# IXarea/LittleGAN

Measured on AMD Instinct MI355X. Metric: 128x128 CelebA-shaped images/sec (G+D+Adj step), higher is better.
Workload: dtype bf16; 1 GPU; C3: 128x128x3 synthetic CelebA, batch 256/GPU, bf16 MFMA conv/transposed-conv + Adjuster branch; global_batch=256, per_gpu_batch=256, image=128, cond_dim=40, parallelism=dp1, launch=eager launches

## Files before the change

littlegan_amd/_lib.py:

```python
from __future__ import annotations

import ctypes as C
import os

_HERE = os.path.dirname(os.path.abspath(__file__))
LIB_PATH = os.path.join(_HERE, "liblittlegan_hip.so")

DT_F32, DT_BF16 = 0, 1

P, I, L, F, Z = C.c_void_p, C.c_int, C.c_longlong, C.c_float, C.c_size_t

SIGNATURES = {
    "lg_abi_version": (I, []),
    "lg_last_error": (C.c_char_p, []),
    "lg_conv_pack_bytes": (Z, [I, I, I]),
    "lg_conv_pack": (I, [P, P, I, I, I, P]),
    "lg_conv2d_s2_fwd": (I, [P, P, P, P, I, I, I, I, I, I, P]),
    "lg_conv_stats_workspace_bytes": (Z, [I, I, I, I, I]),
    "lg_conv_fwd_stats_fused": (I, [I, I, I, I, I, I, I]),
    "lg_conv2d_s2_fwd_stats": (I, [P, P, P, P, P, P, I, I, I, I, I, I, P, Z, P, P]),
    "lg_conv2d_s2_dgrad_m16": (I, [P, P, P, P, P, I, I, I, I, I, I, P]),
    "lg_conv2d_s2_wgrad_m16": (I, [P, P, P, P, P, P, Z, I, I, I, I, I, I, I, P]),
    "lg_conv2d_s2_dgrad": (I, [P, P, P, I, I, I, I, I, I, P]),
    "lg_conv2d_s2_wgrad": (I, [P, P, P, P, Z, I, I, I, I, I, I, I, P]),
# ... 95 lines not shown
    "lg_gp_norm_bwd": (I, [P, P, P, P, P, P, P, P, P, P, P, Z, I, L, F, P]),
    "lg_gp_norm_dd": (I, [P, P, P, P, P, P, P, P, P, P, Z, I, L, F, P]),
    "lg_gp_heads_seed": (I, [P, P, P, I, I, I, P]),
    "lg_gp_heads_2nd": (I, [P, P, P, P, P, P, P, P, I, I, I, P]),
    "lg_diffaug_draw": (I, [P, I, I, I, I, I, P, P]),
    "lg_diffaug_workspace_bytes": (Z, [I, I]),
    "lg_diffaug_fwd": (I, [P, P, P, I, I, P, Z, P]),
    "lg_diffaug_bwd": (I, [P, P, P, I, I, P, Z, P]),
    "lg_rescale_u8": (I, [P, P, I, L, P, P]),
    "lg_soft_labels": (I, [P, P, P, I, I, I, P, P]),
    "lg_augment_drawn_u8_workspace_bytes": (Z, [I]),
    "lg_augment_drawn_u8": (I, [P, P, P, P, I, I, I, F, F, F, F, F, L, L, L, P, Z, P]),
    "lgx_diffaug_draw_gated": (I, [P, I, I, I, I, I, P, P, P]),
    "lgx_ada_init": (I, [P, F, P]),
    "lgx_ada_accumulate": (I, [P, P, I, I, P]),
    "lgx_ada_adjust": (I, [P, I, F, F, P]),
    "lgr_r1_workspace_bytes": (Z, [I, L]),
    "lgr_r1_heads_seed": (I, [P, P, I, I, P]),
    "lgr_r1_seed": (I, [P, P, P, P, P, F, P, Z, I, L, P]),
    "lgr_r1_colsum_workspace_bytes": (Z, [I, I]),
    "lgr_r1_heads_colsum": (I, [P, P, P, Z, I, I, P]),
    "lgo_heads_fwd": (I, [P, P, P, P, P, P, P, P, Z, I, I, I, P]),
    "lgo_gan_heads_loss_fwd_bwd": (I, [P, P, P, I, I, F, F, P, P, I, I, I, P]),
}


GEOM_SIGNATURES = {
    "lgeo_draw": (I, [P, I, I, I, I, I, P, P, P]),
    "lgeo_fwd": (I, [P, P, P, I, I, P]),
    "lgeo_bwd": (I, [P, P, P, I, I, P]),
}


class LittleGanHipError(RuntimeError):
    pass


_lib = None


def load():
    global _lib
    if _lib is not None:
        return _lib
    if not os.path.exists(LIB_PATH):
        raise LittleGanHipError(
            f"{LIB_PATH} not found: build it with `python -m littlegan_amd.csrc.build` "
            "(the LittleGAN hot path has no CPU fallback)")
    from .csrc import build as _build
    variant = os.environ.get("LG_LIB_VARIANT") or None
    path = _build.variant_paths(variant)[1]
    if variant is None:
        fl = _build.built_flags()
        if fl is not None and fl != " ".join(_build.FLAGS):
            raise LittleGanHipError(f"{LIB_PATH} was built with non-default flags ({fl!r}); rebuild with `python -m littlegan_amd.csrc.build`")
    elif not os.path.exists(path):
        raise LittleGanHipError(f"{path} not found: build it with LG_EXTRA_FLAGS=... python -m littlegan_amd.csrc.build --variant {variant}")
    import torch
    lib = C.CDLL(path)
    for name, (res, args) in list(SIGNATURES.items()) + list(GEOM_SIGNATURES.items()):
        fn = getattr(lib, name)
        fn.restype = res
        fn.argtypes = args
    if lib.lg_abi_version() != 1:
        raise LittleGanHipError("liblittlegan_hip.so ABI version mismatch")
    _lib = lib
    return lib


def check(rc: int, what: str):
    if rc != 0:
        msg = load().lg_last_error().decode("utf-8", "replace")
        raise LittleGanHipError(f"{what} failed (rc={rc}): {msg}")
```

littlegan_amd/csrc/build.py:

```python
import glob
import os
import subprocess
import sys
from concurrent.futures import ThreadPoolExecutor

HERE = os.path.dirname(os.path.abspath(__file__))
PKG = os.path.dirname(HERE)
SOURCES = ["capi.hip", "conv_igemm.hip", "conv_halo.hip", "conv_down3.hip", "conv_up3.hip", "n3_kernels.hip", "n3_pgemm.hip", "wgrad_igemm.hip", "pack.hip", "norm.hip", "dense.hip", "heads.hip", "loss_optim.hip", "augment.hip", "fid.hip", "fid_sqrt.hip", "wgrad_at.hip", "wgrad_at32.hip", "n3_rows.hip", "skinny_mfma.hip", "conv_up4.hip", "runtime.hip", "gp.hip", "input_u8.hip", "diffaug.hip", "pairs.hip", "ada.hip", "r1.hip", "objective.hip", "geom.hip"]
LIB = os.path.join(PKG, "liblittlegan_hip.so")
FLAGS = ["--offload-arch=gfx950", "-O3", "-fPIC", "-std=c++17", "-ffp-contract=off", "-Wall", "-Wno-unused-function",
         "-Wmissing-prototypes", "-Werror=missing-prototypes", "-Xclang", "-target-feature", "-Xclang", "-packed-fp32-ops"]


def _stale(out, deps):
    if not os.path.exists(out):
        return True
    t = os.path.getmtime(out)
    return any(os.path.getmtime(d) > t for d in deps)


def variant_paths(variant):
    if not variant:
        return os.path.join(HERE, "build"), LIB
    return os.path.join(HERE, "build_" + variant), os.path.join(PKG, f"liblittlegan_hip_{variant}.so")


def build(force=False, verbose=True, variant=None):
    hipcc = os.environ.get("HIPCC", "/opt/rocm/bin/hipcc")
    objdir, LIB = variant_paths(variant)
    if not variant and os.environ.get("LG_EXTRA_FLAGS"):
        raise SystemExit("LG_EXTRA_FLAGS needs --variant NAME: ablation builds never replace the product library")
    os.makedirs(objdir, exist_ok=True)
    inc = os.path.join(os.path.dirname(PKG), "include")
    headers = sorted(glob.glob(os.path.join(HERE, "*.h"))) + sorted(glob.glob(os.path.join(inc, "littlegan_hip*.h"))) + \
        [os.path.join(inc, "littlegan_geom.h")]

    flags = FLAGS + os.environ.get("LG_EXTRA_FLAGS", "").split()
    flag_line = " ".join(flags)
    only = [s_ for s_ in os.environ.get("LG_VARIANT_SOURCES", "").split(",") if s_] if variant else []
    base_objdir = os.path.join(HERE, "build")

    def cc(src):
        s = os.path.join(HERE, src)
        if only and src not in only:
            o = os.path.join(base_objdir, src.replace(".hip", ".o"))
            if not os.path.exists(o):
                raise SystemExit(f"{o} missing: build the product library first")
            return o
        o = os.path.join(objdir, src.replace(".hip", ".o"))
        fl = o + ".flags"
        same_flags = os.path.exists(fl) and open(fl).read() == flag_line
        if force or not same_flags or _stale(o, [s] + headers):
            cmd = [hipcc] + flags + ["-c", s, "-o", o]
            if verbose:
                print(" ".join(cmd), flush=True)
            if os.path.exists(fl):
                os.remove(fl)
            subprocess.run(cmd, check=True)
            with open(fl, "w") as f:
                f.write(flag_line)
        return o

    with ThreadPoolExecutor(max_workers=6) as ex:
        objs = list(ex.map(cc, SOURCES))
    lib_fl = os.path.join(objdir, "lib.flags")
    if force or _stale(LIB, objs) or not (os.path.exists(lib_fl) and open(lib_fl).read() == flag_line):
        cmd = [hipcc, "--offload-arch=gfx950", "-shared", "-fPIC", "-o", LIB] + objs
        if verbose:
# ... 16 lines not shown
```

littlegan_amd/csrc/norm.hip:

```cpp
#include <stdio.h>
#include "lg_internal.h"
#include "philox.h"

namespace {

constexpr int CHUNK = 4096;
constexpr int EW_UNR = 4;

__global__ __launch_bounds__(256) void stats_partial_kernel(const float* __restrict__ x, double* __restrict__ partial,
                                                            long long L, int nchunk, int pre_leaky, float alpha,
                                                            __bf16* __restrict__ x16out) {
  const int n = blockIdx.y, ch = blockIdx.x;
  const long long base = (long long)n * L + (long long)ch * CHUNK;
  const long long lim = L - (long long)ch * CHUNK;
  __shared__ double sred[32];
  f32x4 v[4];
  double s = 0.0;
  int cnt = 0;
#pragma unroll
  for (int q = 0; q < 4; ++q) {
    const int e = (q * 256 + threadIdx.x) * 4;
    v[q] = f32x4{0.f, 0.f, 0.f, 0.f};
    if (e < lim) {
      v[q] = *reinterpret_cast<const f32x4*>(x + base + e);
// ... 231 lines not shown
  const double* p = partial + (long long)n * nchunk * 2;
  double s1 = 0.0, s2 = 0.0;
  for (int i = lane; i < nchunk; i += 64) { s1 += p[i * 2]; s2 += p[i * 2 + 1]; }
  s1 = lg_wave_sum_d(s1); s2 = lg_wave_sum_d(s2);
  if (lane == 0) {
    const double sigma = (double)stats[(long long)n * LG_NSTAT + 1], s = sigma + (double)LG_IN_EPS;
    const double m1 = s1 / (double)L, m2 = s2 / (double)L / (s * sigma);
    const float m1h = (float)m1, m2h = (float)m2;
    bstats[n * 4] = m1h; bstats[n * 4 + 1] = m2h;
    bstats[n * 4 + 2] = (float)(m1 - (double)m1h); bstats[n * 4 + 3] = (float)(m2 - (double)m2h);
    gsum[n * 2] = s2 / s;
    gsum[n * 2 + 1] = s1;
  }
}

__global__ __launch_bounds__(64) void bwd_coef_kernel(const double* __restrict__ partial, const float* __restrict__ stats,
                                                      float* __restrict__ coef, long long L, int nchunk) {
  const int n = blockIdx.x, lane = threadIdx.x;
  const double* p = partial + (long long)n * nchunk * 2;
  double s1 = 0.0, s2 = 0.0;
  for (int i = lane; i < nchunk; i += 64) { s1 += p[i * 2]; s2 += p[i * 2 + 1]; }
  s1 = lg_wave_sum_d(s1); s2 = lg_wave_sum_d(s2);
  if (lane == 0) {
    const float* sp = stats + (long long)n * LG_NSTAT;
    const double sigma = (double)sp[1], s = sigma + (double)LG_IN_EPS;
    const double m1 = s1 / (double)L, m2 = s2 / (double)L / (s * sigma);
    const float m1h = (float)m1, m2h = (float)m2;
    float* o = coef + (long long)n * 8;
    o[0] = sp[0]; o[1] = sp[4]; o[2] = sp[2]; o[3] = sp[3];
    o[4] = m1h; o[5] = m2h; o[6] = (float)(m1 - (double)m1h); o[7] = (float)(m2 - (double)m2h);
  }
}

__global__ __launch_bounds__(256) void bwd_affine_grad_kernel(const double* __restrict__ gsum, float* __restrict__ dgamma,
                                                              float* __restrict__ dbeta, int B, int accumulate) {
  __shared__ double sg[256], sb[256];
  double g = 0.0, b = 0.0;
  for (int i = threadIdx.x; i < B; i += 256) { g += gsum[i * 2]; b += gsum[i * 2 + 1]; }
  sg[threadIdx.x] = g; sb[threadIdx.x] = b;
  __syncthreads();
  for (int o = 128; o > 0; o >>= 1) {
    if (threadIdx.x < o) { sg[threadIdx.x] += sg[threadIdx.x + o]; sb[threadIdx.x] += sb[threadIdx.x + o]; }
    __syncthreads();
  }
  if (threadIdx.x == 0) {
    dgamma[0] = (accumulate ? dgamma[0] : 0.f) + (float)sg[0];
    dbeta[0] = (accumulate ? dbeta[0] : 0.f) + (float)sb[0];
  }
}

template <bool DB, bool DROP>
__device__ __forceinline__ void bwd_apply_body(const float* __restrict__ x, const void* __restrict__ g, int g16,
                                               const float* __restrict__ stats, const float* __restrict__ bstats,
                                               float* __restrict__ dx, __bf16* __restrict__ dx16, long long L4,
                                               long long total4, int pre_leaky, int post_leaky, float alpha,
                                               float* __restrict__ colpart, int C4, const DropK& dk, const Geo ge) {
  const DropCtx dc = drop_begin<DROP>(dk);
  constexpr int UNR = DB ? 1 : EW_UNR;
  const unsigned stride = ge.gdx * ge.bdx * UNR, tot = (unsigned)total4, l4 = (unsigned)L4;
  f32x4 csum = {0.f, 0.f, 0.f, 0.f};
  const unsigned rb = blockIdx.x;
  const int ntrip = (int)(((unsigned long long)tot + stride - 1) / stride);
  for (int tr = 0; tr < ntrip; ++tr) {
   const unsigned long long i0l = (unsigned long long)tr * stride + rb * ge.bdx * UNR + threadIdx.x;
   if (i0l >= tot) continue;
   const unsigned i0 = (unsigned)i0l;
   f32x4 xs[UNR], gs[UNR];
#pragma unroll
   for (int u = 0; u < UNR; ++u) {
     const unsigned i = i0 + u * 256;
     if (i < tot) {
       xs[u] = lg_ld<NT_LOAD>(reinterpret_cast<const f32x4*>(x + (long long)i * 4));
       gs[u] = load_g4<NT_LOAD>(g, (long long)i * 4, g16);
     }
   }
#pragma unroll
   for (int u = 0; u < UNR; ++u) {
    const unsigned i = i0 + u * 256;
    if (i >= tot) break;
    const int n = (int)(i / l4);
    const float* sp = stats + (long long)n * LG_NSTAT;
// ... 365 lines not shown
    }
  }
}

template <bool DB, bool G16>
__global__ __launch_bounds__(256) void bwd_apply16_kernel(const __bf16* __restrict__ x, const void* __restrict__ g,
                                                          const float* __restrict__ stats, const float* __restrict__ bstats,
                                                          float* __restrict__ dx, __bf16* __restrict__ dx16, long long L8,
                                                          long long total8, int pre_leaky, int post_leaky, float alpha,
                                                          float* __restrict__ colpart, int C8) {
  bwd_apply16_body<DB, G16, false>(x, g, stats, bstats, dx, dx16, L8, total8, pre_leaky, post_leaky, alpha, colpart, C8, DropK{}, Geo{blockDim.x, gridDim.x, gridDim.y});
}
template <bool DB, bool G16>
__global__ __launch_bounds__(256) void bwd_apply16_drop_kernel(const __bf16* __restrict__ x, const void* __restrict__ g,
                                                               const float* __restrict__ stats, const float* __restrict__ bstats,
                                                               float* __restrict__ dx, __bf16* __restrict__ dx16, long long L8,
                                                               long long total8, float alpha, float* __restrict__ colpart, int C8,
                                                               DropK dk) {
  bwd_apply16_body<DB, G16, true>(x, g, stats, bstats, dx, dx16, L8, total8, 0, 1, alpha, colpart, C8, dk, Geo{blockDim.x, gridDim.x, gridDim.y});
}

__global__ __launch_bounds__(256) void dropout_mask_kernel(unsigned char* __restrict__ keep, long long total8, DropK dk) {
  const DropCtx dc = drop_begin<true>(dk);
  for (long long i = (long long)blockIdx.x * 256 + threadIdx.x; i < total8; i += (long long)gridDim.x * 256) {
    float dm[8];
    drop_mult8(dc, (unsigned long long)i, dm);
    unsigned lo = 0, hi = 0;
#pragma unroll
    for (int k = 0; k < 4; ++k) { lo |= (dm[k] != 0.f ? 1u : 0u) << (8 * k); hi |= (dm[4 + k] != 0.f ? 1u : 0u) << (8 * k); }
    *reinterpret_cast<unsigned long long*>(keep + i * 8) = (unsigned long long)lo | ((unsigned long long)hi << 32);
  }
}

__global__ __launch_bounds__(1024) void colsum_final_kernel(const float* __restrict__ partial, float* __restrict__ db, int nb,
                                                            int C, int accumulate) {
  __shared__ float sr[64][17];
  const int cl = threadIdx.x & 15, gq = threadIdx.x >> 4;
  const int c = blockIdx.x * 16 + cl;
  float s = 0.f;
  if (c < C) {
    int k = gq;
    for (; k + 192 < nb; k += 256) {
      const float a = partial[(long long)k * C + c], b = partial[(long long)(k + 64) * C + c];
      const float e = partial[(long long)(k + 128) * C + c], f = partial[(long long)(k + 192) * C + c];
      s += (a + b) + (e + f);
    }
    for (; k < nb; k += 64) s += partial[(long long)k * C + c];
  }
  sr[gq][cl] = s;
  __syncthreads();
  if (gq == 0 && c < C) {
    float t = 0.f;
#pragma unroll
    for (int q = 0; q < 64; q += 4) t += (sr[q][cl] + sr[q + 1][cl]) + (sr[q + 2][cl] + sr[q + 3][cl]);
    db[c] = (accumulate ? db[c] : 0.f) + t;
  }
}

constexpr long long EW_MAX_BLOCKS = 8192;
#define LG_RESIDENT_BLOCKS(kern)                                                                                       \
  ([]() -> long long {                                                                                                 \
    static long long r = 0;                                                                                            \
    if (!r) {                                                                                                          \
      int per_cu = 0;                                                                                                  \
      if (hipOccupancyMaxActiveBlocksPerMultiprocessor(&per_cu, kern, 256, 0) != hipSuccess || per_cu < 1) per_cu = 8; \
      r = (long long)per_cu * lg_device_cus();                                                                         \
    }                                                                                                                  \
    return r;                                                                                                          \
  }())
inline long long fit_rounds(long long nb, long long resident, long long hard, int unit) {
  if (nb > hard) nb = hard;
  if (nb > resident) nb = nb / resident * resident;
  nb = nb / unit * unit;
  return nb < unit ? unit : nb;
}
inline int nchunks(long long L) { return (int)((L + CHUNK - 1) / CHUNK); }
inline int ew_blocks(long long total4) {
  long long b = (total4 + 256 * EW_UNR - 1) / (256 * EW_UNR);
  return (int)(b < EW_MAX_BLOCKS ? (b > 0 ? b : 1) : EW_MAX_BLOCKS);
}
inline size_t part_bytes(int B, long long L) { return ((size_t)B * nchunks(L) * 3 * sizeof(double) + 255) / 256 * 256; }
inline size_t bst_bytes(int B) { return ((size_t)B * 4 * sizeof(float) + 255) / 256 * 256; }

struct LaunchNote { const char* name; unsigned gx, gy; };
constexpr int NL_MAX = 8;
thread_local LaunchNote g_nl[NL_MAX];
thread_local int g_nl_n = 0;
inline void nl_reset() { g_nl_n = 0; }
inline void nl_note(const char* name, const dim3& g) {
// ... 398 lines not shown

extern "C" int lg_dropout_key(long long* key, unsigned long long seed, unsigned long long key_offset, void* stream) {
  nl_reset();
  LG_CHECK_ARG(key && ((uintptr_t)key & 7) == 0, "lg_dropout_key: null or misaligned pointer");
  NORM_LAUNCH(dropout_key_kernel, dim3(1), dim3(64), 0, (hipStream_t)stream, reinterpret_cast<unsigned long long*>(key), seed, key_offset);
  LG_CHECK_LAUNCH("lg_dropout_key");
  return LG_OK;
}

extern "C" int lg_dropout_mask(const long long* key, int call, int level, int r0, int B, long long L, float rate, unsigned char* keep,
                               void* stream) {
  nl_reset();
  LG_CHECK_ARG(keep, "lg_dropout_mask: null pointer");
  LG_CHECK_ARG(((uintptr_t)keep & 7) == 0, "lg_dropout_mask: keep must be 8-byte aligned (8 decisions per store)");
  LG_CHECK_ARG(B > 0 && L > 0 && (long long)B * L / 8 < (1LL << 31), "lg_dropout_mask: bad shape B=%d L=%lld", B, L);
  DropK dk;
  if (int rc = drop_args("lg_dropout_mask", key, call, level, r0, B, L, rate, &dk)) return rc;
  const long long total8 = (long long)B * L / 8;
  long long nb = (total8 + 255) / 256;
  if (nb > EW_MAX_BLOCKS) nb = EW_MAX_BLOCKS;
  NORM_LAUNCH(dropout_mask_kernel, dim3((int)nb), dim3(256), 0, (hipStream_t)stream, keep, total8, dk);
  LG_CHECK_LAUNCH("lg_dropout_mask");
  return LG_OK;
}

extern "C" int lg_instnorm_bwd_coef(const float* stats, const void* partials, int nparts, float* coef, int B, long long L,
                                    void* stream) {
  nl_reset();
  LG_CHECK_ARG(stats && partials && coef && nparts > 0 && B > 0 && B <= 65535 && L > 0, "lg_instnorm_bwd_coef: bad arguments");
  NORM_LAUNCH(bwd_coef_kernel, dim3(B), dim3(64), 0, (hipStream_t)stream, (const double*)partials, stats, coef, L, nparts);
  LG_CHECK_LAUNCH("lg_instnorm_bwd_coef");
  return LG_OK;
}
```

littlegan_amd/model.py:

```python
from __future__ import annotations

import math
import zlib
from typing import Dict, List, Optional

import torch

from . import ops
from ._lib import DT_BF16, DT_F32


def _dtype_of(args) -> int:
    name = getattr(args, "mfma_dtype", "f32")
    if name not in ("f32", "bf16"):
        raise ValueError(f"mfma_dtype must be 'f32' or 'bf16', got {name!r}")
    return DT_BF16 if name == "bf16" else DT_F32


def _device_of(args):
    return torch.device(getattr(args, "device", "cuda"))


def _glorot(shape, gen, device):
    if len(shape) == 2:
# ... 133 lines not shown
        r0 = 0
        if drops is not None and rows is not None:
            r0, _, step = rows.indices(ctx["enc"][0][1].shape[0])
            if step != 1:
                raise ValueError("Encoder.backward: contiguous row ranges only")
        masked = drops is not None and drops[0].active
        g_h = g_last
        levels = set(range(1, 5)) if (need_wgrad and wgrad_levels is None) else (set(wgrad_levels or ()) if need_wgrad else set())
        lowest = 1 if need_input_grad else (min(levels) if levels else 5)
        any_wgrad = need_wgrad
        nfp = None
        for i in range(4, lowest - 1, -1):
            need_wgrad = any_wgrad and i in levels
            cb, cs = self.chans[i - 1]
            x, z, st, x16 = ctx["enc"][i - 1]
            if need_wgrad and x is None and x16 is None:
                raise ValueError("Encoder.backward: this context was recorded with top_only=True (no normalised inputs kept): "
                                 "it cannot give weight gradients")
            if rows is not None:
                z, st = z[rows], st[rows]
                x = x[rows] if x is not None else None
                x16 = x16[rows] if x16 is not None else None
            dgm = self._g[f"norm{i}.gamma"] if need_wgrad else None
            dbt = self._g[f"norm{i}.beta"] if need_wgrad else None
            want_dx = i > lowest or (i == 1 and need_input_grad)
            m16 = self.dtype == DT_BF16
            if cb != 3:
                dz16 = torch.empty(z.shape, dtype=torch.bfloat16, device=z.device) if m16 else None
                drop32 = (m16 and (not need_wgrad or x16 is not None) and
                          (not want_dx or ops.conv_halo_supported(1, self.dtype, z.shape[0], z.shape[1], z.shape[2], cs, cb)))
            else:
                drop32 = m16 and ops.n3_m16_supported(z.shape[1], z.shape[2], cb, cs, self.dtype)
                dz16 = torch.empty(z.shape, dtype=torch.bfloat16, device=z.device) if drop32 else None
            dz = ops.instnorm_bwd(z, st, g_h, dgm, dbt, 0, 1, a, out16=dz16, want_f32=not drop32,
                                  db=self._g[f"conv{i}.bias"] if need_wgrad else None,
                                  partials=nfp, drop=drops[i - 1].at(r0=r0) if drops is not None else None)
            nfp = None
            if need_wgrad:
                ops.conv2d_s2_wgrad(x, dz, self._g[f"conv{i}.kernel"], False, self.dtype, x16=x16, dy16=dz16)
            if not want_dx:
                g_h = None
            elif m16 and i > 1 and drop32 and i - 1 >= lowest and not masked:
                zl, stl = ctx["enc"][i - 2][1], ctx["enc"][i - 2][2]
                if rows is not None:
                    zl, stl = zl[rows], stl[rows]
                g_h, nfp = ops.conv2d_s2_dgrad(None, packs[i - 1], cb, self.dtype, dy16=dz16, out_bf16=True, fuse=(zl, stl, a))
            else:
                g_h = ops.conv2d_s2_dgrad(dz, packs[i - 1], cb, self.dtype, dy16=dz16, out_bf16=(self.dtype == DT_BF16 and i > 1))
        return g_h if need_input_grad else None

    def backward_recorded(self, ctx, g_last):
        a = self.args.leaky_alpha
        packs = self.packs()
        rec = {}
        g_h = g_last
        for i in range(4, 0, -1):
            cb, _ = self.chans[i - 1]
            _, z, st, _ = ctx["enc"][i - 1]
            dz = ops.gp_norm_bwd(z, st, self._w[f"norm{i}.gamma"], g_h, a)
            rec[i] = (g_h, dz)
            g_h = ops.conv2d_s2_dgrad(dz, packs[i - 1], cb, self.dtype)
        return g_h, rec

    def gp_sweep(self, ctx, rec, u0, levels, lowest):
        a = self.args.leaky_alpha
        packs = self.packs()
        u_h, uz2 = u0, {}
        for i in range(1, 5):
            _, cs = self.chans[i - 1]
# ... 81 lines not shown
                h = ops.instnorm_apply(z, st, skip, 0, 1, a, out16=h16, want_f32=not drop32)
            st = ops.stats_tensor(st)
            saved.append((x, z, st, x16))
            x, x16 = h, h16
        if ctx is not None:
            ctx["dec"] = saved
        return x, x16

    def backward(self, ctx, g_h, need_wgrad: bool, wgrad_levels=None, need_input_grad: bool = True, partials=None):
        a = self.args.leaky_alpha
        packs = self.packs()
        levels = set(range(1, 5)) if (need_wgrad and wgrad_levels is None) else (set(wgrad_levels or ()) if need_wgrad else set())
        lowest = 1 if need_input_grad else (min(levels) if levels else 5)
        any_wgrad = need_wgrad
        nfp = partials
        for i in range(4, lowest - 1, -1):
            need_wgrad = any_wgrad and i in levels
            cb, cs = self.chans[i - 1]
            x, z, st, x16 = ctx["dec"][i - 1]
            dgm = self._g[f"norm{i}.gamma"] if need_wgrad else None
            dbt = self._g[f"norm{i}.beta"] if need_wgrad else None
            want_dx = i > lowest or (i == 1 and need_input_grad)
            if (not need_wgrad and want_dx and i > 1 and i - 1 >= lowest and nfp is not None and self.dtype == DT_BF16
                    and z.dtype == torch.bfloat16 and g_h.dtype == torch.bfloat16
                    and ops.convT_s2_dgrad_bn_supported(z.shape[0], z.shape[1] // 2, z.shape[2] // 2, cb, cs, self.dtype)):
                coef = ops.instnorm_bwd_coef(z, st, nfp)
                zl, stl = ctx["dec"][i - 2][1], ctx["dec"][i - 2][2]
                g_h, nfp = ops.convT_s2_dgrad_bn(z, g_h, coef, a, packs[i - 1], cs, fuse=(zl, stl, a))
                continue
            dz16 = torch.empty(z.shape, dtype=torch.bfloat16, device=z.device) if self.dtype == DT_BF16 else None
            drop32 = (dz16 is not None and (not need_wgrad or x16 is not None) and
                      ops.conv_halo_supported(0, self.dtype, z.shape[0], z.shape[1] // 2, z.shape[2] // 2, cb, cs))
            dz = ops.instnorm_bwd(z, st, g_h, dgm, dbt, 0, 1, a, out16=dz16, want_f32=not drop32,
                                  db=self._g[f"conv{i}.bias"] if need_wgrad else None, partials=nfp)
            nfp = None
            if need_wgrad:
                ops.convT_s2_wgrad(x, dz, self._g[f"conv{i}.kernel"], False, self.dtype, x16=x16, dy16=dz16)
            if not want_dx:
                g_h = None
            elif dz16 is not None and drop32 and i > 1 and i - 1 >= lowest:
                zl, stl = ctx["dec"][i - 2][1], ctx["dec"][i - 2][2]
                g_h, nfp = ops.convT_s2_dgrad(None, packs[i - 1], cs, self.dtype, dy16=dz16, out_bf16=True, fuse=(zl, stl, a))
            else:
                g_h = ops.convT_s2_dgrad(dz, packs[i - 1], cs, self.dtype, dy16=dz16, out_bf16=self.dtype == DT_BF16)
        return g_h if need_input_grad else None


class _FinalConv(_Module):

    def __init__(self, args):
        super().__init__(args)
        self.cb, self.cs = args.image_channel, args.conv_filter[4]
        self._add("kernel", (5, 5, self.cb, self.cs), "kernel")
        self._add("bias", (self.cb,), "zeros")
        self._pack = None
        self._pack_version = -1
        self.version = 0

    def pack(self):
        if self._pack_version != self.version:
            self._pack = ops.conv_pack(self._w["kernel"], self.cb, self.cs, self.dtype, out=self._pack)
            self._pack_version = self.version
        return self._pack

    def __call__(self, x, out=None, x16=None):
        return ops.convT_s1_tanh_fwd(x, self.pack(), self._w["bias"], self.cb, self.dtype, out=out, x16=x16)

# ... 328 lines not shown
```

littlegan_amd/ops.py:

```python
from __future__ import annotations

import torch

from . import _lib
from ._lib import DT_BF16, DT_F32, check

_WS = {}
_WS_RETIRED = []
_WS_PINNED = False
NSTAT = 8


class Profile:
    enabled = False
    records = []
    after_conv = None

    @classmethod
    def start(cls):
        cls.records = []
        cls.enabled = True

    @classmethod
    def stop(cls):
# ... 530 lines not shown
    if drop is not None:
        lib = _lib.load()
        if pend is not None:
            m = pend.m
            part = m.ws.data_ptr() + pend.lo * m.nparts * 3 * 8
            check(lib.lg_instnorm_leaky_apply_z16_p_drop(_p(x), part, m.nparts, _p(m.gamma), _p(m.beta), _p(stats), _p(out), _p(out16), B, Ln,
                                                         float(alpha), *drop._args(), _stream()), "lg_instnorm_leaky_apply_z16_p_drop")
            m.covered += B
        elif x_is16:
            check(lib.lg_instnorm_leaky_apply_z16_drop(_p(x), _p(stats), _p(out), _p(out16), B, Ln, float(alpha), *drop._args(), _stream()),
                  "lg_instnorm_leaky_apply_z16_drop")
        else:
            check(lib.lg_instnorm_leaky_apply_drop(_p(x), _p(stats), _p(out), _p(out16), B, Ln, float(alpha), *drop._args(), _stream()),
                  "lg_instnorm_leaky_apply_drop")
        return out
    if pend is not None:
        m = pend.m
        part = m.ws.data_ptr() + pend.lo * m.nparts * 3 * 8
        check(_lib.load().lg_instnorm_leaky_apply_z16_p(_p(x), part, m.nparts, _p(m.gamma), _p(m.beta), _p(stats), _p(skip), int(skip16),
                                                        _p(out), _p(out16), B, Ln, int(post_leaky), float(alpha), _stream()),
              "lg_instnorm_leaky_apply_z16_p")
        m.covered += B
    elif x_is16:
        check(_lib.load().lg_instnorm_leaky_apply_z16(_p(x), _p(stats), _p(skip), int(skip16), _p(out), _p(out16), B, Ln,
                                                      int(pre_leaky), int(post_leaky), float(alpha), _stream()),
              "lg_instnorm_leaky_apply_z16")
    else:
        check(_lib.load().lg_instnorm_leaky_apply(_p(x), _p(stats), _p(skip), _p(out), _p(out16), B, Ln, int(pre_leaky),
                                                  int(post_leaky), float(alpha), _stream()), "lg_instnorm_leaky_apply")
    return out


def instnorm_bwd(x, stats, g, dgamma, dbeta, pre_leaky, post_leaky, alpha, accumulate=False, out=None, out16=None,
                 want_f32=True, db=None, partials=None, drop=None):
    B = x.shape[0]
    Ln = x.numel() // B
    x_is16 = x.dtype == torch.bfloat16
    if x_is16:
        _chk16(x, x, "x")
        if Ln % 8:
            raise ValueError("instnorm_bwd: a bf16 input needs a multiple of 8 elements per sample")
    else:
        _chk(x, name="x")
    if drop is not None:
        _chk_drop(drop, "instnorm_bwd", None, pre_leaky, post_leaky, Ln)
        if partials is not None and drop.active:
            raise ValueError("instnorm_bwd: producer-fused partial sums are those of the unmasked gradient; with an active dropout "
                             "mask the first pass must run (partials=None)")
    g16 = g.dtype == torch.bfloat16
    if g16:
        _chk16(g, x, "g")
    else:
        _chk(g, name="g")
        if g.numel() != x.numel():
            raise ValueError("instnorm_bwd: g has a different size")
    _chk(stats, (B, NSTAT), "stats")
    if want_f32:
        if out is None:
            out = torch.empty(x.shape, dtype=torch.float32, device=x.device)
        _chk(out, x.shape, "out")
    else:
        if out16 is None:
            raise ValueError("instnorm_bwd: want_f32=False needs out16")
        out = None
    if out16 is not None:
        _chk16(out16, x, "out16")
    lib = _lib.load()
# ... 4 lines not shown
    ws = workspace(int(lib.lg_instnorm_bwd_db_workspace_bytes(B, Ln, C)), x.device, "small")
    if partials is not None:
        if not x_is16:
            raise ValueError("instnorm_bwd: fused partial sums belong to the bf16 activation path")
        if pre_leaky or not post_leaky or float(alpha) != partials.alpha or tuple(x.shape) != partials.shape:
            raise ValueError(f"instnorm_bwd: partial sums were produced for the post-LeakyReLU(alpha={partials.alpha}) form on "
                             f"shape {partials.shape}; asked for pre={pre_leaky} post={post_leaky} alpha={alpha} shape {tuple(x.shape)}")
        if drop is not None:
            check(lib.lg_instnorm_leaky_bwd_z16_drop(_p(x), _p(stats), _p(g), int(g16), _p(out), _p(out16), _p(dgamma), _p(dbeta), _p(db), C,
                                                     _p(partials.buf), int(partials.nparts), _p(ws), ws.numel(), B, Ln, float(alpha),
                                                     int(accumulate), *drop._args(), _stream()), "lg_instnorm_leaky_bwd_z16_drop")
            return out
        check(lib.lg_instnorm_leaky_bwd_z16_p(_p(x), _p(stats), _p(g), int(g16), _p(out), _p(out16), _p(dgamma), _p(dbeta), _p(db), C,
                                              _p(partials.buf), int(partials.nparts), _p(ws), ws.numel(), B, Ln, int(pre_leaky),
                                              int(post_leaky), float(alpha), int(accumulate), _stream()),
              "lg_instnorm_leaky_bwd_z16_p")
        return out
    if drop is not None:
        if x_is16:
            check(lib.lg_instnorm_leaky_bwd_z16_drop(_p(x), _p(stats), _p(g), int(g16), _p(out), _p(out16), _p(dgamma), _p(dbeta), _p(db), C,
                                                     None, 0, _p(ws), ws.numel(), B, Ln, float(alpha), int(accumulate), *drop._args(),
                                                     _stream()), "lg_instnorm_leaky_bwd_z16_drop")
        else:
            check(lib.lg_instnorm_leaky_bwd_drop(_p(x), _p(stats), _p(g), int(g16), _p(out), _p(out16), _p(dgamma), _p(dbeta), _p(db), C,
                                                 _p(ws), ws.numel(), B, Ln, float(alpha), int(accumulate), *drop._args(), _stream()),
                  "lg_instnorm_leaky_bwd_drop")
        return out
    fn = lib.lg_instnorm_leaky_bwd_z16 if x_is16 else lib.lg_instnorm_leaky_bwd_db
    check(fn(_p(x), _p(stats), _p(g), int(g16), _p(out), _p(out16), _p(dgamma), _p(dbeta), _p(db), C, _p(ws), ws.numel(), B, Ln,
             int(pre_leaky), int(post_leaky), float(alpha), int(accumulate), _stream()), "lg_instnorm_leaky_bwd")
    return out


def dense_fwd(x, w, bias, out=None):
    B, K = x.shape
    N = w.shape[1]
    _chk(x, name="x")
    _chk(w, (K, N), "w")
    if out is None:
        out = torch.empty(B, N, dtype=torch.float32, device=x.device)
    _chk(out, (B, N), "out")
    check(_lib.load().lg_dense_fwd(_p(x), _p(w), _p(bias), _p(out), B, K, N, _stream()), "lg_dense_fwd")
    return out


def dense_wgrad(x, dy, dw, db, accumulate=False):
    B, K = x.shape
    N = dy.shape[1]
    _chk(x, name="x")
    _chk(dy, (B, N), "dy")
    _chk(dw, (K, N), "dw")
    check(_lib.load().lg_dense_wgrad(_p(x), _p(dy), _p(dw), _p(db), B, K, N, int(accumulate), _stream()),
          "lg_dense_wgrad")


def concat_cols(a, c, out=None):
    B, ka = a.shape
    kc = c.shape[1]
    _chk(a, name="a")
    _chk(c, (B, kc), "c")
    if out is None:
        out = torch.empty(B, ka + kc, dtype=torch.float32, device=a.device)
    _chk(out, (B, ka + kc), "out")
    check(_lib.load().lg_concat_cols(_p(a), ka, _p(c), kc, _p(out), B, _stream()), "lg_concat_cols")
    return out

# ... 782 lines not shown
```

Baseline: 24800 images/sec.

## Fold instance-norm backward reductions into apply kernel and merge bias/affine tail

Adds a new instance-norm backward path for bf16 inputs. The apply kernel reduces the per-sample partial sums itself, writes the affine-gradient partials and the column bias partials, and reverses its traversal order so the most recently touched data is read first. A single tail kernel then finishes both the bias column sums and the dgamma/dbeta reduction. The aim is fewer launches and fewer separate reduction passes in the discriminator and generator backward. Each apply block now repeats the partial-sum reduction, and the path is used only when dropout is inactive.

Result: no change. 24990 images/sec (median of 6 runs) (+0.8%).

```diff
diff --git a/include/littlegan_normbwd.h b/include/littlegan_normbwd.h
--- /dev/null
+++ b/include/littlegan_normbwd.h
@@ -0,0 +1,20 @@
+#ifndef LITTLEGAN_NORMBWD_H
+#define LITTLEGAN_NORMBWD_H
+#include "littlegan_hip.h"
+
+#ifdef __cplusplus
+extern "C" {
+#endif
+
+int lgnb_bwd_z16_supported(int B, long long L, int C);
+int lgnb_plan_gx(int B, long long L, int C, long long resident);
+long long lgnb_resident_blocks(int db, int g_is_bf16);
+size_t lgnb_workspace_bytes(int B, long long L, int C);
+int lgnb_bwd_z16(const void* z16, const float* stats, const void* g, int g_is_bf16, float* dx, void* dx16, float* dgamma, float* dbeta,
+                 float* db, int C, const void* partials, int nparts_in, void* workspace, size_t ws_bytes, int B, long long L,
+                 int pre_leaky, int post_leaky, float alpha, int accumulate, void* stream);
+
+#ifdef __cplusplus
+}
+#endif
+#endif
diff --git a/littlegan_amd/_lib.py b/littlegan_amd/_lib.py
--- a/littlegan_amd/_lib.py
+++ b/littlegan_amd/_lib.py
@@ -151,6 +151,15 @@
 }
 
 
+NORMBWD_SIGNATURES = {
+    "lgnb_bwd_z16_supported": (I, [I, L, I]),
+    "lgnb_plan_gx": (I, [I, L, I, L]),
+    "lgnb_resident_blocks": (L, [I, I]),
+    "lgnb_workspace_bytes": (Z, [I, L, I]),
+    "lgnb_bwd_z16": (I, [P, P, P, I, P, P, P, P, P, I, P, I, P, Z, I, L, I, I, F, I, P]),
+}
+
+
 class LittleGanHipError(RuntimeError):
     pass
 
@@ -177,7 +186,7 @@
         raise LittleGanHipError(f"{path} not found: build it with LG_EXTRA_FLAGS=... python -m littlegan_amd.csrc.build --variant {variant}")
     import torch
     lib = C.CDLL(path)
-    for name, (res, args) in list(SIGNATURES.items()) + list(GEOM_SIGNATURES.items()):
+    for name, (res, args) in list(SIGNATURES.items()) + list(GEOM_SIGNATURES.items()) + list(NORMBWD_SIGNATURES.items()):
         fn = getattr(lib, name)
         fn.restype = res
         fn.argtypes = args
diff --git a/littlegan_amd/csrc/build.py b/littlegan_amd/csrc/build.py
--- a/littlegan_amd/csrc/build.py
+++ b/littlegan_amd/csrc/build.py
@@ -33,7 +33,7 @@
     os.makedirs(objdir, exist_ok=True)
     inc = os.path.join(os.path.dirname(PKG), "include")
     headers = sorted(glob.glob(os.path.join(HERE, "*.h"))) + sorted(glob.glob(os.path.join(inc, "littlegan_hip*.h"))) + \
-        [os.path.join(inc, "littlegan_geom.h")]
+        [os.path.join(inc, "littlegan_geom.h"), os.path.join(inc, "littlegan_normbwd.h")]
 
     flags = FLAGS + os.environ.get("LG_EXTRA_FLAGS", "").split()
     flag_line = " ".join(flags)
diff --git a/littlegan_amd/csrc/norm.hip b/littlegan_amd/csrc/norm.hip
--- a/littlegan_amd/csrc/norm.hip
+++ b/littlegan_amd/csrc/norm.hip
@@ -287,12 +287,14 @@
   }
 }
 
-__global__ __launch_bounds__(256) void bwd_affine_grad_kernel(const double* __restrict__ gsum, float* __restrict__ dgamma,
-                                                              float* __restrict__ dbeta, int B, int accumulate) {
+__device__ __forceinline__ void bwd_affine_grad_body(const double* __restrict__ gsum, float* __restrict__ dgamma,
+                                                     float* __restrict__ dbeta, int B, int accumulate) {
   __shared__ double sg[256], sb[256];
-  double g = 0.0, b = 0.0;
-  for (int i = threadIdx.x; i < B; i += 256) { g += gsum[i * 2]; b += gsum[i * 2 + 1]; }
-  sg[threadIdx.x] = g; sb[threadIdx.x] = b;
+  if (threadIdx.x < 256) {
+    double g = 0.0, b = 0.0;
+    for (int i = threadIdx.x; i < B; i += 256) { g += gsum[i * 2]; b += gsum[i * 2 + 1]; }
+    sg[threadIdx.x] = g; sb[threadIdx.x] = b;
+  }
   __syncthreads();
   for (int o = 128; o > 0; o >>= 1) {
     if (threadIdx.x < o) { sg[threadIdx.x] += sg[threadIdx.x + o]; sb[threadIdx.x] += sb[threadIdx.x + o]; }
@@ -302,6 +304,10 @@
     dgamma[0] = (accumulate ? dgamma[0] : 0.f) + (float)sg[0];
     dbeta[0] = (accumulate ? dbeta[0] : 0.f) + (float)sb[0];
   }
+}
+__global__ __launch_bounds__(256) void bwd_affine_grad_kernel(const double* __restrict__ gsum, float* __restrict__ dgamma,
+                                                              float* __restrict__ dbeta, int B, int accumulate) {
+  bwd_affine_grad_body(gsum, dgamma, dbeta, B, accumulate);
 }
 
 template <bool DB, bool DROP>
@@ -733,8 +739,8 @@
   }
 }
 
-__global__ __launch_bounds__(1024) void colsum_final_kernel(const float* __restrict__ partial, float* __restrict__ db, int nb,
-                                                            int C, int accumulate) {
+__device__ __forceinline__ void colsum_final_body(const float* __restrict__ partial, float* __restrict__ db, int nb, int C,
+                                                  int accumulate) {
   __shared__ float sr[64][17];
   const int cl = threadIdx.x & 15, gq = threadIdx.x >> 4;
   const int c = blockIdx.x * 16 + cl;
@@ -756,6 +762,10 @@
     for (int q = 0; q < 64; q += 4) t += (sr[q][cl] + sr[q + 1][cl]) + (sr[q + 2][cl] + sr[q + 3][cl]);
     db[c] = (accumulate ? db[c] : 0.f) + t;
   }
+}
+__global__ __launch_bounds__(1024) void colsum_final_kernel(const float* __restrict__ partial, float* __restrict__ db, int nb,
+                                                            int C, int accumulate) {
+  colsum_final_body(partial, db, nb, C, accumulate);
 }
 
 constexpr long long EW_MAX_BLOCKS = 8192;
@@ -1220,3 +1230,5 @@
   LG_CHECK_LAUNCH("lg_instnorm_bwd_coef");
   return LG_OK;
 }
+
+#include "norm_bwd_p.h"
diff --git a/littlegan_amd/csrc/norm_bwd_p.h b/littlegan_amd/csrc/norm_bwd_p.h
--- /dev/null
+++ b/littlegan_amd/csrc/norm_bwd_p.h
@@ -0,0 +1,219 @@
+#pragma once
+#include "../../include/littlegan_normbwd.h"
+
+namespace {
+
+constexpr int NBP_TRIPS = 2;
+
+template <bool DB, bool G16>
+__global__ __launch_bounds__(256) void bwd_apply16p_kernel(const __bf16* __restrict__ x, const void* __restrict__ g,
+                                                           const float* __restrict__ stats, const double* __restrict__ partial,
+                                                           int nchunk, double* __restrict__ gsum, float* __restrict__ dx,
+                                                           __bf16* __restrict__ dx16, unsigned L8, long long L, int pre_leaky,
+                                                           int post_leaky, float alpha, float* __restrict__ colpart, int C8) {
+  const Geo ge{blockDim.x, gridDim.x, gridDim.y};
+  constexpr int UNR = DB ? DB_UNR : EW8_UNR;
+  __shared__ float sbs[4];
+  const int n = (int)(ge.gdy - 1 - blockIdx.y);
+  const unsigned bx = ge.gdx - 1 - blockIdx.x;
+  const unsigned ustep = DB ? ge.gdx * ge.bdx : 256u;
+  const unsigned stride = ge.gdx * ge.bdx * UNR;
+  const unsigned first = DB ? bx * ge.bdx + threadIdx.x : bx * ge.bdx * UNR + threadIdx.x;
+  const long long base = (long long)n * L8;
+  const int ntrip = (int)((L8 + stride - 1) / stride);
+  f32x8 xs[UNR], gs[UNR];
+  unsigned i0 = (unsigned)(ntrip - 1) * stride + first;
+#pragma unroll
+  for (int u = 0; u < UNR; ++u) {
+    const unsigned i = i0 + u * ustep;
+    if (i < L8) { xs[u] = load8<true, NT_LOAD>(x, base + i); gs[u] = load8<G16, NT_LOAD>(g, base + i); }
+  }
+  const float* sp = stats + (long long)n * LG_NSTAT;
+  const float mu = sp[0], a = sp[2], b = sp[3], mul = sp[4];
+  if (threadIdx.x < 64) {
+    const int lane = threadIdx.x;
+    const double* p = partial + (long long)n * nchunk * 2;
+    double s1 = 0.0, s2 = 0.0;
+    for (int i = lane; i < nchunk; i += 64) { s1 += p[i * 2]; s2 += p[i * 2 + 1]; }
+    s1 = lg_wave_sum_d(s1); s2 = lg_wave_sum_d(s2);
+    if (lane == 0) {
+      const double sigma = (double)sp[1], s = sigma + (double)LG_IN_EPS;
+      const double m1 = s1 / (double)L, m2 = s2 / (double)L / (s * sigma);
+      const float m1h = (float)m1, m2h = (float)m2;
+      sbs[0] = m1h; sbs[1] = m2h;
+      sbs[2] = (float)(m1 - (double)m1h); sbs[3] = (float)(m2 - (double)m2h);
+      if (bx == 0) {
+        gsum[n * 2] = s2 / s;
+        gsum[n * 2 + 1] = s1;
+      }
+    }
+  }
+  __syncthreads();
+  const float m1 = sbs[0], m2 = sbs[1], m1l = sbs[2], m2l = sbs[3];
+  f32x8 csum;
+  csum.lo = f32x4{0.f, 0.f, 0.f, 0.f}; csum.hi = f32x4{0.f, 0.f, 0.f, 0.f};
+  for (int tr = 0; tr < ntrip; ++tr) {
+    if (tr > 0) {
+      i0 = (unsigned)(ntrip - 1 - tr) * stride + first;
+#pragma unroll
+      for (int u = 0; u < UNR; ++u) {
+        const unsigned i = i0 + u * ustep;
+        if (i < L8) { xs[u] = load8<true, NT_LOAD>(x, base + i); gs[u] = load8<G16, NT_LOAD>(g, base + i); }
+      }
+    }
+#pragma unroll
+    for (int u = 0; u < UNR; ++u) {
+      const unsigned i = i0 + u * ustep;
+      if (i >= L8) break;
+      f32x8 o;
+#pragma unroll
+      for (int k = 0; k < 8; ++k) {
+        const float x0 = k < 4 ? xs[u].lo[k & 3] : xs[u].hi[k & 3];
+        float xx = x0;
+        if (pre_leaky) xx = lg_leaky(xx, alpha);
+        const float c = (xx - mu) - mul;
+        float dz = k < 4 ? gs[u].lo[k & 3] : gs[u].hi[k & 3];
+        if (post_leaky) dz = (a * c + b > 0.f) ? dz : alpha * dz;
+        float d = a * ((((dz - m1) - m1l) - c * m2) - c * m2l);
+        if (pre_leaky) d = (x0 > 0.f) ? d : alpha * d;
+        if (k < 4) o.lo[k & 3] = d; else o.hi[k & 3] = d;
+      }
+      if (dx) store8_f32(dx, base + i, o);
+      if (dx16) store8_bf16(dx16, base + i, o);
+      if constexpr (DB) { csum.lo += o.lo; csum.hi += o.hi; }
+    }
+  }
+  if constexpr (DB) {
+    __shared__ f32x4 sacc[512];
+    sacc[2 * threadIdx.x] = csum.lo; sacc[2 * threadIdx.x + 1] = csum.hi;
+    __syncthreads();
+    const int q = threadIdx.x;
+    if (q < C8) {
+      const int cb = (int)(((long long)bx * 256) % C8);
+      const long long row = (long long)n * ge.gdx + bx;
+      f32x4 tl = {0.f, 0.f, 0.f, 0.f}, th = {0.f, 0.f, 0.f, 0.f};
+      for (int k = (q - cb + C8) % C8; k < 256; k += C8) { tl += sacc[2 * k]; th += sacc[2 * k + 1]; }
+      *reinterpret_cast<f32x4*>(colpart + (row * C8 + q) * 8) = tl;
+      *reinterpret_cast<f32x4*>(colpart + (row * C8 + q) * 8 + 4) = th;
+    }
+  }
+}
+
+__global__ __launch_bounds__(1024) void bwd_tail_kernel(const float* __restrict__ colpart, float* __restrict__ db, int nb, int C,
+                                                        const double* __restrict__ gsum, float* __restrict__ dgamma,
+                                                        float* __restrict__ dbeta, int B, int accumulate) {
+  if (blockIdx.x + 1 == gridDim.x)
+    bwd_affine_grad_body(gsum, dgamma, dbeta, B, accumulate);
+  else
+    colsum_final_body(colpart, db, nb, C, accumulate);
+}
+
+inline size_t nbp_gsum_bytes(int B) { return ((size_t)B * 2 * sizeof(double) + 255) / 256 * 256; }
+inline int nbp_unit(int C) { return 256 % (C / 8) == 0 ? 1 : 3; }
+inline bool nbp_c_ok(long long L, int C) {
+  return C > 0 && C % 8 == 0 && C / 8 <= 256 && L % C == 0 && (256 % (C / 8) == 0 || 768 % (C / 8) == 0);
+}
+inline bool nbp_shape_ok(int B, long long L) { return B > 0 && B <= 65535 && L > 0 && L % 8 == 0 && (long long)B * L / 8 < (1LL << 31); }
+
+}
+
+extern "C" int lgnb_bwd_z16_supported(int B, long long L, int C) {
+  if (!nbp_shape_ok(B, L)) return 0;
+  if (C == 0) return 1;
+  return nbp_c_ok(L, C) && (long long)B * nbp_unit(C) <= DB_MAX_BLOCKS;
+}
+
+extern "C" int lgnb_plan_gx(int B, long long L, int C, long long resident) {
+  if (!lgnb_bwd_z16_supported(B, L, C) || resident < 1) return 0;
+  const long long L8 = L / 8, unr = 256 * (C ? DB_UNR : EW8_UNR) * NBP_TRIPS;
+  long long gx = (L8 + unr - 1) / unr;
+  long long cap = (C ? (long long)DB_MAX_BLOCKS : EW_MAX_BLOCKS) / B;
+  if (cap < 1) cap = 1;
+  if (gx > cap) gx = cap;
+  if (gx * B > resident) {
+    gx = gx * B / resident * resident / B;
+    if (gx < 1) gx = 1;
+  }
+  if (C) {
+    const int unit = nbp_unit(C);
+    gx = gx / unit * unit;
+    if (gx < unit) gx = unit;
+  }
+  return (int)gx;
+}
+
+extern "C" long long lgnb_resident_blocks(int db, int g_is_bf16) {
+  if (db) return g_is_bf16 ? LG_RESIDENT_BLOCKS((bwd_apply16p_kernel<true, true>)) : LG_RESIDENT_BLOCKS((bwd_apply16p_kernel<true, false>));
+  return g_is_bf16 ? LG_RESIDENT_BLOCKS((bwd_apply16p_kernel<false, true>)) : LG_RESIDENT_BLOCKS((bwd_apply16p_kernel<false, false>));
+}
+
+extern "C" size_t lgnb_workspace_bytes(int B, long long L, int C) {
+  if (B < 1 || L < 1) return 0;
+  return part_bytes(B, L) + nbp_gsum_bytes(B) + (C > 0 ? (size_t)DB_MAX_BLOCKS * (size_t)C * sizeof(float) : 0);
+}
+
+extern "C" int lgnb_bwd_z16(const void* z16, const float* stats, const void* g, int g_is_bf16, float* dx, void* dx16, float* dgamma,
+                            float* dbeta, float* db, int C, const void* partials, int nparts_in, void* workspace, size_t ws_bytes, int B,
+                            long long L, int pre_leaky, int post_leaky, float alpha, int accumulate, void* stream) {
+  nl_reset();
+  LG_CHECK_ARG(z16 && stats && g && (dx || dx16) && workspace, "lgnb_bwd_z16: null pointer");
+  LG_CHECK_ARG(!dgamma == !dbeta, "lgnb_bwd_z16: dgamma and dbeta come together");
+  LG_CHECK_ARG(nbp_shape_ok(B, L), "lgnb_bwd_z16: bad shape B=%d L=%lld", B, L);
+  LG_CHECK_ARG(!(partials && nparts_in > 0) || (pre_leaky == 0 && post_leaky == 1),
+               "lgnb_bwd_z16: fused partial sums exist for pre_leaky=0, post_leaky=1 only (got %d, %d)", pre_leaky, post_leaky);
+  if (!db) C = 0;
+  if (db) {
+    LG_CHECK_ARG(nbp_c_ok(L, C), "lgnb_bwd_z16: unsupported channel count C=%d (L=%lld)", C, L);
+    LG_CHECK_ARG(lgnb_bwd_z16_supported(B, L, C), "lgnb_bwd_z16: unsupported shape: %d samples leave no whole block row of the column partials (C=%d)", B, C);
+  }
+  LG_CHECK_ARG(ws_bytes >= lgnb_workspace_bytes(B, L, C), "lgnb_bwd_z16: workspace too small");
+  hipStream_t st = (hipStream_t)stream;
+  const __bf16* x = (const __bf16*)z16;
+  char* ws = (char*)workspace;
+  const double* partial = (const double*)ws;
+  double* gsum = (double*)(ws + part_bytes(B, L));
+  float* colpart = (float*)(ws + part_bytes(B, L) + nbp_gsum_bytes(B));
+  int nc = nparts_in;
+  if (partials && nparts_in > 0) {
+    partial = (const double*)partials;
+  } else {
+    nc = 4096 / B;
+    if (nc < 1) nc = 1;
+    const int nch8 = (int)((L + 2 * CHUNK - 1) / (2 * CHUNK));
+    if (nc > nch8) nc = nch8;
+    if (g_is_bf16)
+      NORM_LAUNCH(bwd_partial16_kernel<true>, dim3(nc, B), dim3(256), 0, st, x, g, stats, (double*)ws, L, nc, pre_leaky, post_leaky, alpha);
+    else
+      NORM_LAUNCH(bwd_partial16_kernel<false>, dim3(nc, B), dim3(256), 0, st, x, g, stats, (double*)ws, L, nc, pre_leaky, post_leaky, alpha);
+    LG_CHECK_LAUNCH("lgnb_bwd_z16(partial)");
+  }
+  const int gx = lgnb_plan_gx(B, L, C, lgnb_resident_blocks(db != nullptr, g_is_bf16));
+  const dim3 grid((unsigned)gx, (unsigned)B);
+  const unsigned L8 = (unsigned)(L / 8);
+  if (db && g_is_bf16)
+    NORM_LAUNCH((bwd_apply16p_kernel<true, true>), grid, dim3(256), 0, st, x, g, stats, partial, nc, gsum, dx, (__bf16*)dx16, L8, L,
+                pre_leaky, post_leaky, alpha, colpart, C / 8);
+  else if (db)
+    NORM_LAUNCH((bwd_apply16p_kernel<true, false>), grid, dim3(256), 0, st, x, g, stats, partial, nc, gsum, dx, (__bf16*)dx16, L8, L,
+                pre_leaky, post_leaky, alpha, colpart, C / 8);
+  else if (g_is_bf16)
+    NORM_LAUNCH((bwd_apply16p_kernel<false, true>), grid, dim3(256), 0, st, x, g, stats, partial, nc, gsum, dx, (__bf16*)dx16, L8, L,
+                pre_leaky, post_leaky, alpha, (float*)nullptr, 0);
+  else
+    NORM_LAUNCH((bwd_apply16p_kernel<false, false>), grid, dim3(256), 0, st, x, g, stats, partial, nc, gsum, dx, (__bf16*)dx16, L8, L,
+                pre_leaky, post_leaky, alpha, (float*)nullptr, 0);
+  LG_CHECK_LAUNCH("lgnb_bwd_z16(apply)");
+  lg_note_kernel(db ? "bwd_apply16p_kernel<DB>" : "bwd_apply16p_kernel");
+  if (db && dgamma) {
+    NORM_LAUNCH(bwd_tail_kernel, dim3((C + 15) / 16 + 1), dim3(1024), 0, st, (const float*)colpart, db, gx * B, C, (const double*)gsum,
+                dgamma, dbeta, B, accumulate);
+    LG_CHECK_LAUNCH("lgnb_bwd_z16(tail)");
+  } else if (db) {
+    NORM_LAUNCH(colsum_final_kernel, dim3((C + 15) / 16), dim3(1024), 0, st, (const float*)colpart, db, gx * B, C, accumulate);
+    LG_CHECK_LAUNCH("lgnb_bwd_z16(bias)");
+  } else if (dgamma) {
+    NORM_LAUNCH(bwd_affine_grad_kernel, dim3(1), dim3(256), 0, st, (const double*)gsum, dgamma, dbeta, B, accumulate);
+    LG_CHECK_LAUNCH("lgnb_bwd_z16(affine)");
+  }
+  return LG_OK;
+}
diff --git a/littlegan_amd/model.py b/littlegan_amd/model.py
--- a/littlegan_amd/model.py
+++ b/littlegan_amd/model.py
@@ -189,9 +189,11 @@
             else:
                 drop32 = m16 and ops.n3_m16_supported(z.shape[1], z.shape[2], cb, cs, self.dtype)
                 dz16 = torch.empty(z.shape, dtype=torch.bfloat16, device=z.device) if drop32 else None
-            dz = ops.instnorm_bwd(z, st, g_h, dgm, dbt, 0, 1, a, out16=dz16, want_f32=not drop32,
-                                  db=self._g[f"conv{i}.bias"] if need_wgrad else None,
-                                  partials=nfp, drop=drops[i - 1].at(r0=r0) if drops is not None else None)
+            db = self._g[f"conv{i}.bias"] if need_wgrad else None
+            drop = drops[i - 1].at(r0=r0) if drops is not None else None
+            fold = (drop is None or not drop.active) and ops.instnorm_bwd_p_supported(z, db=need_wgrad)
+            dz = ops.instnorm_bwd(z, st, g_h, dgm, dbt, 0, 1, a, out16=dz16, want_f32=not drop32, db=db,
+                                  partials=nfp, drop=None if fold else drop, fold=fold)
             nfp = None
             if need_wgrad:
                 ops.conv2d_s2_wgrad(x, dz, self._g[f"conv{i}.kernel"], False, self.dtype, x16=x16, dy16=dz16)
@@ -339,7 +341,8 @@
             drop32 = (dz16 is not None and (not need_wgrad or x16 is not None) and
                       ops.conv_halo_supported(0, self.dtype, z.shape[0], z.shape[1] // 2, z.shape[2] // 2, cb, cs))
             dz = ops.instnorm_bwd(z, st, g_h, dgm, dbt, 0, 1, a, out16=dz16, want_f32=not drop32,
-                                  db=self._g[f"conv{i}.bias"] if need_wgrad else None, partials=nfp)
+                                  db=self._g[f"conv{i}.bias"] if need_wgrad else None, partials=nfp,
+                                  fold=ops.instnorm_bwd_p_supported(z, db=need_wgrad))
             nfp = None
             if need_wgrad:
                 ops.convT_s2_wgrad(x, dz, self._g[f"conv{i}.kernel"], False, self.dtype, x16=x16, dy16=dz16)
diff --git a/littlegan_amd/ops.py b/littlegan_amd/ops.py
--- a/littlegan_amd/ops.py
+++ b/littlegan_amd/ops.py
@@ -586,7 +586,12 @@
 
 
 def instnorm_bwd(x, stats, g, dgamma, dbeta, pre_leaky, post_leaky, alpha, accumulate=False, out=None, out16=None,
-                 want_f32=True, db=None, partials=None, drop=None):
+                 want_f32=True, db=None, partials=None, drop=None, fold=False):
+    if fold:
+        if drop is not None:
+            raise ValueError("instnorm_bwd: fold=True knows no dropout mask")
+        return instnorm_bwd_p(x, stats, g, dgamma, dbeta, pre_leaky, post_leaky, alpha, accumulate=accumulate, out=out, out16=out16,
+                              want_f32=want_f32, db=db, partials=partials)
     B = x.shape[0]
     Ln = x.numel() // B
     x_is16 = x.dtype == torch.bfloat16
@@ -657,6 +662,58 @@
     return out
 
 
+def instnorm_bwd_p_supported(x, db=False):
+    B = x.shape[0]
+    return bool(x.dtype == torch.bfloat16 and _lib.load().lgnb_bwd_z16_supported(B, x.numel() // B, x.shape[-1] if db else 0))
+
+
+def instnorm_bwd_p(x, stats, g, dgamma, dbeta, pre_leaky, post_leaky, alpha, accumulate=False, out=None, out16=None,
+                   want_f32=True, db=None, partials=None):
+    B = x.shape[0]
+    Ln = x.numel() // B
+    if x.dtype != torch.bfloat16:
+        raise ValueError("instnorm_bwd_p: x must be the bf16 conv output (the fp32 path is instnorm_bwd's)")
+    _chk16(x, x, "x")
+    if Ln % 8:
+        raise ValueError("instnorm_bwd_p: a bf16 input needs a multiple of 8 elements per sample")
+    g16 = g.dtype == torch.bfloat16
+    if g16:
+        _chk16(g, x, "g")
+    else:
+        _chk(g, name="g")
+        if g.numel() != x.numel():
+            raise ValueError("instnorm_bwd_p: g has a different size")
+    _chk(stats, (B, NSTAT), "stats")
+    if want_f32:
+        if out is None:
+            out = torch.empty(x.shape, dtype=torch.float32, device=x.device)
+        _chk(out, x.shape, "out")
+    else:
+        if out16 is None:
+            raise ValueError("instnorm_bwd_p: want_f32=False needs out16")
+        out = None
+    if out16 is not None:
+        _chk16(out16, x, "out16")
+    if (dgamma is None) != (dbeta is None):
+        raise ValueError("instnorm_bwd_p: dgamma and dbeta come together")
+    lib = _lib.load()
+    C = 0
+    if db is not None:
+        C = x.shape[-1]
+        _chk(db, (C,), "db")
+    nparts = 0
+    if partials is not None:
+        if pre_leaky or not post_leaky or float(alpha) != partials.alpha or tuple(x.shape) != partials.shape:
+            raise ValueError(f"instnorm_bwd_p: partial sums were produced for the post-LeakyReLU(alpha={partials.alpha}) form on "
+                             f"shape {partials.shape}; asked for pre={pre_leaky} post={post_leaky} alpha={alpha} shape {tuple(x.shape)}")
+        nparts = int(partials.nparts)
+    ws = workspace(int(lib.lgnb_workspace_bytes(B, Ln, C)), x.device, "small")
+    check(lib.lgnb_bwd_z16(_p(x), _p(stats), _p(g), int(g16), _p(out), _p(out16), _p(dgamma), _p(dbeta), _p(db), C,
+                           _p(partials.buf) if partials is not None else None, nparts, _p(ws), ws.numel(), B, Ln, int(pre_leaky),
+                           int(post_leaky), float(alpha), int(accumulate), _stream()), "lgnb_bwd_z16")
+    return out
+
+
 def dense_fwd(x, w, bias, out=None):
     B, K = x.shape
     N = w.shape[1]
```
